# CHONSPQX/modulated-deform-conv

Measured on AMD Instinct MI355X. Metric: fwd+bwd GSamples/s, MDCN2d 3x3 C=256 56x56 B=32; %HBM roofline, higher is better.
Workload: dtype f32; 1 GPU; ModulatedDeformConv2d 3x3, C_in=C_out=256, 56x56, deformable_group=1, fp32, B=32 per GPU, forward+backward (BASELINE.json configs[1]); global_batch=32, parallelism=dp1 batch-sharded

## Files before the change

modulated_deform_conv_amd/csrc/mfma_bwd_data.hip:

```cpp
#include "mfma_kernels.hpp"
#include "mfma_tile.hpp"
#include <algorithm>
#include <map>
#include <mutex>
#include <stdio.h>
#include <stdlib.h>
#include <type_traits>

namespace mdconv {

namespace {

int grid_for(int64_t total) {
  int64_t b = (total + 255) / 256;
  return (int)(b > 8192 ? 8192 : (b < 1 ? 1 : b));
}

__device__ __forceinline__ void pack_wq_items(const Geom &g, int ochunks, int cblks, const float *__restrict__ w,
                                              float *__restrict__ wq, int64_t first, int64_t step) {
  const int64_t total = (int64_t)g.K * ochunks * cblks * 2 * 64;
  for (int64_t i = first; i < total; i += step) {
    int64_t r = i;
    const int lane = (int)(r & 63); r >>= 6;
    const int q = (int)(r & 1); r >>= 1;
// ... 12 lines not shown
    reinterpret_cast<float4 *>(wq)[i] = make_float4(v[0], v[1], v[2], v[3]);
  }
}

__global__ __launch_bounds__(256) void pack_wq_kernel(Geom g, int ochunks, int cblks,
                                                      const float *__restrict__ w,
                                                      float *__restrict__ wq) {
  pack_wq_items(g, ochunks, cblks, w, wq, (int64_t)blockIdx.x * 256 + threadIdx.x, (int64_t)gridDim.x * 256);
}

__global__ __launch_bounds__(256) void bwd_prep_kernel(Geom g, int ochunks, int cblks, const float *__restrict__ w,
                                                       float *__restrict__ wq, int *__restrict__ cnt, int64_t cnt_n,
                                                       const float *__restrict__ x, float *__restrict__ xt,
                                                       int nb_pack, int nb_zero, int qtiles, int ctiles) {
  __shared__ float t[32][33];
  int bid = blockIdx.x;
  if (bid < nb_pack) {
    pack_wq_items(g, ochunks, cblks, w, wq, (int64_t)bid * 256 + threadIdx.x, (int64_t)nb_pack * 256);
    return;
  }
  bid -= nb_pack;
  if (bid < nb_zero) {
    for (int64_t i = (int64_t)bid * 256 + threadIdx.x; i < cnt_n; i += (int64_t)nb_zero * 256) cnt[i] = 0;
    return;
  }
  bid -= nb_zero;
  const int qx = bid % qtiles, cy = (bid / qtiles) % ctiles, b = bid / (qtiles * ctiles);
  nchw_to_nhwc_tile(t, g.C, g.S_i, x, xt, b, cy * 32, qx * 32);
}




template <int ND, bool MOD, int WAVES_C, int QPQ, bool CL, typename GP = GeomRuntime>
__global__ __launch_bounds__(256, 2) void mfma_bwd_data_kernel(
    Geom g_arg, BwdDims bd, const float *__restrict__ input, const float *__restrict__ gout,
    const float *__restrict__ wq, const float *__restrict__ offset, const float *__restrict__ mask,
    float *__restrict__ gcol, float *__restrict__ grad_offset, float *__restrict__ grad_mask,
    float *__restrict__ ga, float *__restrict__ bias_part, int *__restrict__ cnt,
    int *__restrict__ table, const float *__restrict__ xt, int ntiles, int n_full, int n_tail, int tpw) {
  constexpr int NC = 1 << ND, NP = NC / 2;
  constexpr int MB = 2;
  constexpr int WAVES_P = 4 / WAVES_C;
  constexpr int BNP = 32 * WAVES_P;
  constexpr int RB = ND == 2 ? 8 : 4;
  constexpr int NBATCH = MB * 16 / RB;
  constexpr int HS = NBATCH / 2, CPS = NC / HS;
  constexpr int kOob = 0x7ffffff0;
  static_assert(!GP::kFixed || (ND == 2 && MOD && QPQ > 0), "the canonical geometry is 2-D, modulated, one conv group");
  const auto &g = GP::view(g_arg);
  extern __shared__ __attribute__((aligned(16))) float smem[];
  const int T_o = bd.ochunks;
  const int gpitch = T_o * 16 + 4;
  float *Gs = smem;
  float *red = smem + BNP * gpitch;
  const int kTapGroup = bd.tap_group;

  const int tid = threadIdx.x, lane = tid & 63, kh = lane >> 5;
  const int wave = __builtin_amdgcn_readfirstlane(tid >> 6);
  const int wc = wave / WAVES_P, wp = wave % WAVES_P;

  int u0, u1;
  if ((int)blockIdx.x < n_full) {
    u0 = xcd_remap(blockIdx.x, n_full) * g.K * tpw;
    u1 = u0 + g.K * tpw;
  } else {
    const int j = xcd_remap(blockIdx.x - n_full, n_tail);
    const int64_t tail_units = (int64_t)(ntiles - n_full * tpw) * g.K;
    u0 = n_full * tpw * g.K + (int)(tail_units * j / n_tail);
    u1 = n_full * tpw * g.K + (int)(tail_units * (j + 1) / n_tail);
  }
  if (u0 >= u1) return;

  const int passes = bd.cblks_q / (2 * WAVES_C);
  const int iters = (u1 - u0) * passes;
  const int nquads = T_o / 4;
  const bool per_block = g.DG > 1;
  const int nblk = per_block ? passes * WAVES_C : WAVES_C;
  const int bpd = per_block ? g.Cdg / 64 : nblk;
  const int frag_bytes = 64 * 16;
  const int chunk_bytes = bd.cblks_q * 2 * frag_bytes;
  const rsrc_t r_in = make_rsrc(CL ? xt : input, (size_t)g.B * g.C * g.S_i * 4);
  const rsrc_t r_wq = make_rsrc(wq, (size_t)g.K * T_o * chunk_bytes);
  const rsrc_t r_gc = make_rsrc(gcol, (size_t)g.B * g.C * g.K * g.S_o * 4);
  const int a_lane = lane * 16;
  const float *Bb = Gs + (wp * 32 + (lane & 31)) * gpitch + 4 * kh;
  constexpr int kStRow = 2 * NC + 4;
  float *Pk = red + bd.red_floats + wave * (32 * 64);
  int *St = reinterpret_cast<int *>(red + bd.red_floats + 4 * 32 * 64) + wave * (32 * kStRow);
  const int gl_p = lane >> 2, gl_j = lane & 3;
  auto pk_swz = [](int p) { return ((p & 3) << 2) | ((p >> 2) & 3); };
  if (CL) {
    for (int i = lane; i < 32 * 64; i += 64) Pk[i] = 0.f;
    for (int i = lane; i < 32 * kStRow; i += 64) St[i] = kOob;
  }

  auto krange = [&](int pass, int &q_lo, int &q_n) {
    if (g.G == 1) { q_lo = 0; q_n = nquads; return; }
    const int cb = (pass * WAVES_C + wc) * 64;
    const int c_lo = min(cb, g.C - 1), c_hi = min(cb + 63, g.C - 1);
    const int o_lo = (c_lo / g.Cg) * g.Og, o_hi = (c_hi / g.Cg + 1) * g.Og;
    q_lo = o_lo / 64;
    q_n = (o_hi + 63) / 64 - q_lo;
  };
  auto a_base = [&](int tap, int pass, int q_lo) {
    return (tap * T_o + q_lo * 4) * chunk_bytes + ((pass * WAVES_C + wc) * 2) * 2 * frag_bytes;
  };
  int a_cur = 0, n_cur = 0, a_nxt = 0, b_cur = 0;
  auto a_off = [&](int t) { return t < n_cur ? a_cur + t * chunk_bytes : a_nxt + (t - n_cur) * chunk_bytes; };
  auto load_a = [&](float4 (&ra)[MB][2], int soff) {
#pragma unroll
    for (int i = 0; i < MB; ++i)
#pragma unroll
      for (int q = 0; q < 2; ++q)
        ra[i][q] = buf_load4(r_wq, a_lane + (i * 2 + q) * frag_bytes, soff);
  };
  float4 ra0[MB][2], ra1[MB][2], ra2[MB][2], ra3[MB][2];
  {
    int q_lo, q_n;
    krange(0, q_lo, q_n);
    a_cur = a_base(u0 % g.K, 0, q_lo);
    n_cur = 4;
    load_a(ra0, a_off(0));
    load_a(ra1, a_off(1));
    load_a(ra2, a_off(2));
  }

  struct Pix { int n0, b, pix; bool live; int oc[ND]; };
  auto pix_of_tile = [&](int tile, Pix &px) {
    px.n0 = tile * BNP;
    const int n_raw = px.n0 + wp * 32 + (lane & 31);
    px.live = n_raw < g.N;
    const int n_l = px.live ? n_raw : g.N - 1;
    px.b = n_l / g.S_o;
    px.pix = n_l - px.b * g.S_o;
    out_coords<ND>(g, px.pix, px.oc);
  };
  Pix pc, pp;
  pix_of_tile(u0 / g.K, pc);
  pp = pc;

  auto load_gout_tile = [&](int tile) {
    const int j = tid % BNP, osub = tid / BNP;
    constexpr int OSTEP = 256 / BNP;
    const int n_t = min(tile * BNP + j, g.N - 1);
    const int b_t = n_t / g.S_o, pix_t = n_t - b_t * g.S_o;
    const bool t_live = tile * BNP + j < g.N;
    const float *src = gout + ((int64_t)b_t * g.O) * g.S_o + pix_t;
    float *dst = Gs + j * gpitch;
    const int Opad = T_o * 16;
#pragma unroll 8
    for (int o = osub; o < Opad; o += OSTEP) {
      const float v = src[(int64_t)min(o, g.O - 1) * g.S_o];
      dst[o] = (t_live && o < g.O) ? v : 0.f;
    }
  };

  constexpr int PGS = BNP / 4;
  constexpr int OPR = 256 / PGS;
  constexpr int kPre = 8;
  const bool gout_vec = (g.S_o & 3) == 0 && (reinterpret_cast<uintptr_t>(gout) & 15) == 0;
  auto load_gout_tile_vec = [&](int tile) {
    const int Opad = T_o * 16;
    const int rounds = (Opad + OPR - 1) / OPR;
    const int j4 = (tid % PGS) * 4;
    const bool live4 = tile * BNP + j4 < g.N;
    const int n4 = min(tile * BNP + j4, g.N - 4);
    const int b4 = n4 / g.S_o, pix4 = n4 - b4 * g.S_o;
    const float *src = gout + ((int64_t)b4 * g.O) * g.S_o + pix4;
    const int o0 = tid / PGS;
    float *dst = Gs + j4 * gpitch + o0;
    for (int r0 = 0; r0 < rounds; r0 += kPre) {
      float4 v[kPre];
#pragma unroll
      for (int i = 0; i < kPre; ++i)
        v[i] = *reinterpret_cast<const float4 *>(src + (int64_t)min((r0 + i) * OPR + o0, g.O - 1) * g.S_o);
#pragma unroll
      for (int i = 0; i < kPre; ++i) {
        const int o = (r0 + i) * OPR + o0;
        if (o < Opad) {
          const bool on = live4 && o < g.O;
          float *d = dst + (r0 + i) * OPR;
          d[0] = on ? v[i].x : 0.f;
          d[gpitch] = on ? v[i].y : 0.f;
          d[2 * gpitch] = on ? v[i].z : 0.f;
          d[3 * gpitch] = on ? v[i].w : 0.f;
        }
      }
    }
  };

  auto emit_ga = [&](int tile) {
    constexpr int NCH = BNP / 16;
    const int Opad = T_o * 16;
    const int total = NCH * bd.mblks * 2 * 64;
    for (int i = tid; i < total; i += 256) {
      int r = i;
      const int ln = r & 63; r >>= 6;
      const int q = r & 1; r >>= 1;
      const int mblk = r % bd.mblks, nch = r / bd.mblks;
      const int nchunk = tile * NCH + nch;
      if (nchunk * 16 >= bd.Np) continue;
      const int o = mblk * 32 + (ln & 31);
      const float *src = Gs + (nch * 16 + 8 * q + 4 * (ln >> 5)) * gpitch + o;
      float4 v = make_float4(0.f, 0.f, 0.f, 0.f);
      if (o < Opad) v = make_float4(src[0], src[gpitch], src[2 * gpitch], src[3 * gpitch]);
      reinterpret_cast<float4 *>(ga)[((int64_t)nchunk * bd.mblks + mblk) * 128 + q * 64 + ln] = v;
    }
    if (bias_part != nullptr)
      for (int o = tid; o < g.O; o += 256) {
        float sacc = 0.f;
#pragma unroll 8
        for (int px = 0; px < BNP; ++px) sacc += Gs[px * gpitch + o];
        bias_part[(int64_t)tile * g.O + o] = sacc;
      }
  };

  int voff[NP], gc_voff = kOob;
  int voffc[NC];
  struct Fac { float ol[ND - 1], oh[ND - 1], osl[ND - 1], osh[ND - 1], xw, yw, xs, ys; } fac;
  float mg = 0.f;
  float S[NC];
  float delta_n[ND], m_n = 1.f;
  typedef unsigned long long lanemask_t;
  lanemask_t bad[NC];
#pragma unroll
  for (int ci = 0; ci < NC; ++ci) bad[ci] = 0ull;
  f32x16 acc[MB], accp[MB];
#pragma unroll
  for (int pi = 0; pi < NP; ++pi) voff[pi] = kOob;
#pragma unroll
  for (int ci = 0; ci < NC; ++ci) voffc[ci] = kOob;
#pragma unroll
  for (int ci = 0; ci < NC; ++ci) S[ci] = 0.f;
#pragma unroll
  for (int a = 0; a < ND; ++a) delta_n[a] = 0.f;
#pragma unroll
  for (int a = 0; a < ND - 1; ++a) fac.ol[a] = fac.oh[a] = fac.osl[a] = fac.osh[a] = 0.f;
  fac.xw = fac.yw = fac.xs = fac.ys = 0.f;
#pragma unroll
  for (int i = 0; i < MB; ++i)
#pragma unroll
    for (int r = 0; r < 16; ++r) accp[i][r] = 0.f;

  auto new_tap_state = [&](int tapp, int dgp, bool count) {
    int tcd[ND];
    tap_coords<ND>(g, tapp, tcd);
    TapCoef<ND, float> tc;
    make_tap<ND, float>(g, pp.oc, tcd, delta_n, true, tc);
    mg = (!g.range_gate || tc.inside) ? m_n : 0.f;
    int pidx[NP];
    float px[NP], py[NP];
    make_pairs<ND, float>(g, tc, 1.f, pidx, px, py);
    bool prx[NP], pry[NP];
    make_pairs_read<ND, float>(g, tc, prx, pry);
    if (ND == 3 && count && kh == 0 && pp.live) {
      SampleAnchor<ND> sa;
      sample_anchor<ND>(g, tc, 1.f, sa);
      if (sa.on) atomicAdd(cnt + ((int64_t)pp.b * g.DG + dgp) * bd.S_e + sa.qa, 1);
    }
    if (ND == 2 && count && kh == 0 && pp.live) {
      int aidx[NP];
      float ax[NP], ay[NP];
      make_pairs_f<ND, float>(g, tc, tc.wl, tc.wha, 1.f, aidx, ax, ay);
      int *cseg = cnt + ((int64_t)pp.b * g.DG + dgp) * g.S_i;
#pragma unroll
      for (int pi = 0; pi < NP; ++pi)
        if (ax[pi] != 0.f || ay[pi] != 0.f) atomicAdd(cseg + aidx[pi], 1);
    }
    if (count && kh == 0) {
      const int n = pp.n0 + wp * 32 + lane;
      if (n < bd.Np) {
        int *e = table + ((int64_t)(dgp * g.K + tapp) * bd.Np + n) * (2 * NC);
        int ev[2 * NC];
#pragma unroll
        for (int pi = 0; pi < NP; ++pi) {
          if (bd.cl) {
            ev[2 * pi] = pp.live && prx[pi] ? (pp.b * g.S_i + pidx[pi]) * g.C * 4 : kOob;
// ... 21 lines not shown
      }
      voffc[2 * pi] = prx[pi] ? (pp.b * g.S_i + pidx[pi]) * g.C * 4 + 16 * kh : kOob;
      voffc[2 * pi + 1] = pry[pi] ? (pp.b * g.S_i + pidx[pi] + 1) * g.C * 4 + 16 * kh : kOob;
    }
    {
      constexpr int L = ND - 1;
      const int lc = tc.last_lc, hc = tc.last_lc + tc.delta[L];
      const int cl = min(lc, g.in_sz[L] - 2);
      fac.xw = (lc == cl ? tc.wl[L] : 0.f) + (hc == cl ? tc.wh[L] : 0.f);
      fac.yw = (lc == cl + 1 ? tc.wl[L] : 0.f) + (hc == cl + 1 ? tc.wh[L] : 0.f);
      fac.xs = (lc == cl ? tc.sl[L] : 0.f) + (hc == cl ? tc.sh[L] : 0.f);
      fac.ys = (lc == cl + 1 ? tc.sl[L] : 0.f) + (hc == cl + 1 ? tc.sh[L] : 0.f);
#pragma unroll
      for (int a = 0; a < L; ++a) { fac.ol[a] = tc.wl[a]; fac.oh[a] = tc.wh[a]; fac.osl[a] = tc.sl[a]; fac.osh[a] = tc.sh[a]; }
    }
    gc_voff = pp.live ? ((((pp.b * g.K + tapp) * g.S_o + pp.pix) * g.C) + 4 * kh) * 4 : kOob;
    if (CL && kh == 0) {
      int *st = St + lane * kStRow;
#pragma unroll
      for (int c4 = 0; c4 < NC; c4 += 4)
        *reinterpret_cast<int4 *>(st + c4) = make_int4(voffc[c4], voffc[c4 + 1], voffc[c4 + 2], voffc[c4 + 3]);
      st[NC] = gc_voff;
    }
#pragma unroll
    for (int ci = 0; ci < NC; ++ci) S[ci] = 0.f;
  };

  struct Batch { float f[RB * NC]; };
  auto gather = [&](int q, int cbase_p, Batch &v) {
    const int mb = (q * RB) / 16, r0 = (q * RB) % 16;
    if (CL) {
      const int pxl = (q / HS) * 16 + gl_p;
      const int *st = St + pxl * kStRow + (q % HS) * CPS;
      const bool full = cbase_p + 64 <= g.C;
      if (full) {
#pragma unroll
        for (int c = 0; c < CPS; ++c) {
          const int o = st[c] + 16 * gl_j;
#pragma unroll
          for (int k = 0; k < 4; ++k) {
            const float4 x = buf_load4(r_in, o + 64 * k, cbase_p * 4);
            float *d = v.f + (c * 4 + k) * 4;
            d[0] = x.x; d[1] = x.y; d[2] = x.z; d[3] = x.w;
          }
        }
      } else {
#pragma unroll
        for (int c = 0; c < CPS; ++c) {
          const int o = st[c] + 16 * gl_j;
#pragma unroll
          for (int k = 0; k < 4; ++k) {
            const float4 x = buf_load4(r_in, cbase_p + 16 * k + 4 * gl_j < g.C ? o + 64 * k : kOob, cbase_p * 4);
            float *d = v.f + (c * 4 + k) * 4;
            d[0] = x.x; d[1] = x.y; d[2] = x.z; d[3] = x.w;
          }
        }
      }
    } else {
#pragma unroll
      for (int rr = 0; rr < RB; ++rr) {
        const int r = r0 + rr;
        const int cu = cbase_p + mb * 32 + (r & 3) + 8 * (r >> 2);
        const int cs = min(cu, g.C - 5) * g.S_i * 4;
#pragma unroll
        for (int pi = 0; pi < NP; ++pi) {
          const float2 x = buf_load2(r_in, voff[pi], cs);
          v.f[(rr * NP + pi) * 2] = x.x;
          v.f[(rr * NP + pi) * 2 + 1] = x.y;
        }
      }
    }
  };
  auto consume = [&](int q, int cbase_p, const Batch &v) {
    if (CL) {
      const int pxl = (q / HS) * 16 + gl_p, cp = q % HS;
      int *st = St + pxl * kStRow;
      const int swz = pk_swz(pxl);
      const bool full = cbase_p + 64 <= g.C;
      float4 gc[4];
#pragma unroll
      for (int k = 0; k < 4; ++k)
        gc[k] = *reinterpret_cast<const float4 *>(Pk + pxl * 64 + 4 * ((4 * k + gl_j) ^ swz));
      if (cp == 0) {
        const int gv = st[NC] + 16 * gl_j;
#pragma unroll
        for (int k = 0; k < 4; ++k)
          buf_store4(r_gc, (full || cbase_p + 16 * k + 4 * gl_j < g.C) ? gv + 64 * k : kOob, cbase_p * 4,
                     gc[k].x, gc[k].y, gc[k].z, gc[k].w);
      }
      float s[CPS];
#pragma unroll
      for (int c = 0; c < CPS; ++c) {
        float a = 0.f;
#pragma unroll
        for (int k = 0; k < 4; ++k) {
          const float *x = v.f + (c * 4 + k) * 4;
          a = fmaf(gc[k].w, x[3], fmaf(gc[k].z, x[2], fmaf(gc[k].y, x[1], fmaf(gc[k].x, x[0], a))));
        }
        s[c] = a;
      }
      static_assert(CPS == 2, "two corners per step");
      asm("s_nop 1\n\t"
          "v_add_f32_dpp %0, %0, %0 quad_perm:[1,0,3,2] row_mask:0xf bank_mask:0xf\n\t"
          "v_add_f32_dpp %1, %1, %1 quad_perm:[1,0,3,2] row_mask:0xf bank_mask:0xf\n\t"
          "s_nop 1\n\t"
          "v_add_f32_dpp %0, %0, %0 quad_perm:[2,3,0,1] row_mask:0xf bank_mask:0xf\n\t"
          "v_add_f32_dpp %1, %1, %1 quad_perm:[2,3,0,1] row_mask:0xf bank_mask:0xf\n\t"
          "s_nop 1"
          : "+v"(s[0]), "+v"(s[1]));
      if (gl_j == 0) *reinterpret_cast<float2 *>(st + NC + 4 + cp * CPS) = make_float2(s[0], s[1]);
      return;
    }
    const int mb = (q * RB) / 16, r0 = (q * RB) % 16;
#pragma unroll
    for (int gq = 0; gq < RB / 4; ++gq) {
      const int cu4 = cbase_p + mb * 32 + 8 * ((r0 >> 2) + gq);
      const int vo = cu4 < g.C ? gc_voff : kOob;
      buf_store4(r_gc, vo, cu4 * 4, accp[mb][r0 + 4 * gq], accp[mb][r0 + 4 * gq + 1],
                 accp[mb][r0 + 4 * gq + 2], accp[mb][r0 + 4 * gq + 3]);
    }
    lanemask_t any_bad = 0ull;
#pragma unroll
    for (int ci = 0; ci < NC; ++ci) any_bad |= bad[ci];
    if (any_bad != 0ull) {
#pragma unroll
      for (int rr = 0; rr < RB; ++rr) {
        const float gc = accp[mb][r0 + rr];
#pragma unroll
        for (int ci = 0; ci < NC; ++ci) {
          float x;
          asm("v_cndmask_b32_e64 %0, %1, 0, %2" : "=v"(x) : "v"(v.f[(rr * NP + (ci >> 1)) * 2 + (ci & 1)]), "s"(bad[ci]));
          S[ci] = fmaf(gc, x, S[ci]);
        }
      }
    } else {
#pragma unroll
      for (int rr = 0; rr < RB; ++rr) {
        const float gc = accp[mb][r0 + rr];
#pragma unroll
        for (int ci = 0; ci < NC; ++ci) {
          const float x = v.f[(rr * NP + (ci >> 1)) * 2 + (ci & 1)];
          S[ci] = fmaf(gc, x, S[ci]);
        }
      }
    }
#pragma unroll
    for (int ci = 0; ci < NC; ++ci) asm volatile("" : "+v"(S[ci]));
  };

  auto collect = [&]() {
    if (CL) {
      const float *sr = reinterpret_cast<const float *>(St + (lane & 31) * kStRow + NC + 4);
#pragma unroll
      for (int c4 = 0; c4 < NC; c4 += 4) {
        const float4 t = *reinterpret_cast<const float4 *>(sr + c4);
        S[c4] += t.x; S[c4 + 1] += t.y; S[c4 + 2] += t.z; S[c4 + 3] += t.w;
      }
    }
  };
  auto park = [&]() {
    if (CL) {
      const int pix = lane & 31, swz = pk_swz(pix);
      float *dst = Pk + pix * 64;
#pragma unroll
      for (int i = 0; i < MB; ++i)
#pragma unroll
        for (int rq = 0; rq < 4; ++rq)
          *reinterpret_cast<float4 *>(dst + 4 * ((i * 8 + 2 * rq + kh) ^ swz)) =
              make_float4(acc[i][4 * rq], acc[i][4 * rq + 1], acc[i][4 * rq + 2], acc[i][4 * rq + 3]);
    } else {
#pragma unroll
      for (int i = 0; i < MB; ++i) accp[i] = acc[i];
    }
  };

  int grp_lo = (u0 % g.K) % kTapGroup;
  auto finish_tap = [&](int tapp, int blk, bool flush_ok, bool last) {
    float goff[ND], gm = 0.f;
    {
      constexpr int L = ND - 1;
      float Tw[NP], Ts[NP];
#pragma unroll
      for (int pi = 0; pi < NP; ++pi) {
        Tw[pi] = fmaf(fac.xw, S[2 * pi], fac.yw * S[2 * pi + 1]);
        Ts[pi] = fmaf(fac.xs, S[2 * pi], fac.ys * S[2 * pi + 1]);
      }
#pragma unroll
      for (int a = 0; a < ND; ++a) goff[a] = 0.f;
#pragma unroll
      for (int pi = 0; pi < NP; ++pi) {
        float ow = 1.f;
#pragma unroll
        for (int a = 0; a < L; ++a) ow *= ((pi >> (L - 1 - a)) & 1) ? fac.oh[a] : fac.ol[a];
        gm = fmaf(ow, Tw[pi], gm);
        goff[L] = fmaf(ow, Ts[pi], goff[L]);
#pragma unroll
        for (int a = 0; a < L; ++a) {
          float od = 1.f;
#pragma unroll
          for (int a2 = 0; a2 < L; ++a2) {
            const bool hi = (pi >> (L - 1 - a2)) & 1;
            od *= (a2 == a) ? (hi ? fac.osh[a2] : fac.osl[a2]) : (hi ? fac.oh[a2] : fac.ol[a2]);
          }
          goff[a] = fmaf(od, Tw[pi], goff[a]);
        }
      }
#pragma unroll
      for (int a = 0; a < ND; ++a) goff[a] *= mg;
    }
    if (!CL) {
#pragma unroll
      for (int a = 0; a < ND; ++a) goff[a] += __shfl_xor(goff[a], 32, 64);
      gm += __shfl_xor(gm, 32, 64);
    }
    if (bd.red_floats == 0) {
      if (kh == 0 && pp.live) {
        const int64_t ob = ((int64_t)pp.b * (ND * g.K) + ND * tapp) * g.S_o + pp.pix;
#pragma unroll
        for (int a = 0; a < ND; ++a) {
          float *dst = grad_offset + ob + (int64_t)a * g.S_o;
          *dst = g.acc_data ? *dst + goff[a] : goff[a];
        }
        if (MOD) {
          float *dst = grad_mask + ((int64_t)pp.b * g.K + tapp) * g.S_o + pp.pix;
          *dst = g.acc_data ? *dst + gm : gm;
        }
      }
      return;
    }
    const int slot = tapp % kTapGroup;
    if (kh == 0) {
      float *rp = red + ((slot * nblk + blk) * (ND + 1)) * BNP + wp * 32 + lane;
#pragma unroll
      for (int a = 0; a < ND; ++a) rp[a * BNP] = goff[a];
      rp[ND * BNP] = gm;
    }
    if (flush_ok && (slot == kTapGroup - 1 || tapp == g.K - 1 || last)) {
      __syncthreads();
      const int tap0 = tapp - slot;
      const int per_slot = g.DG * (ND + 1) * BNP;
      const int items = (slot + 1 - grp_lo) * per_slot;
      for (int x = tid; x < items; x += 256) {
        const int jj = x % BNP, a = (x / BNP) % (ND + 1), dgi = (x / (BNP * (ND + 1))) % g.DG;
        const int sl = grp_lo + x / per_slot;
        const int n = pp.n0 + jj;
        if (n < g.N && (MOD || a < ND)) {
          float sum = 0.f;
          for (int y = 0; y < bpd; ++y)
            sum += red[((sl * nblk + dgi * bpd + y) * (ND + 1) + a) * BNP + jj];
          const int b = n / g.S_o, pix = n - b * g.S_o, tp = tap0 + sl;
          const int64_t seg = (int64_t)b * g.DG + dgi;
          float *dst = a < ND ? grad_offset + (seg * (ND * g.K) + ND * tp + a) * g.S_o + pix
                              : grad_mask + (seg * g.K + tp) * g.S_o + pix;
          *dst = g.acc_data ? *dst + sum : sum;
        }
      }
      __syncthreads();
      grp_lo = 0;
    }
  };

  auto mma = [&](const float4 (&ra)[MB][2], const float *bp, bool fresh) {
    const float4 b0 = *reinterpret_cast<const float4 *>(bp);
    const float4 b1 = *reinterpret_cast<const float4 *>(bp + 8);
    const f32x16 zero = {0.f, 0.f, 0.f, 0.f, 0.f, 0.f, 0.f, 0.f, 0.f, 0.f, 0.f, 0.f, 0.f, 0.f, 0.f, 0.f};
#pragma unroll
    for (int q = 0; q < 2; ++q)
#pragma unroll
      for (int s = 0; s < 4; ++s) {
        const float4 bq = q == 0 ? b0 : b1;
        const float b = s == 0 ? bq.x : (s == 1 ? bq.y : (s == 2 ? bq.z : bq.w));
#pragma unroll
        for (int i = 0; i < MB; ++i) {
          const float a = s == 0 ? ra[i][q].x : (s == 1 ? ra[i][q].y : (s == 2 ? ra[i][q].z : ra[i][q].w));
          acc[i] = __builtin_amdgcn_mfma_f32_32x32x2f32(a, b, (fresh && q == 0 && s == 0) ? zero : acc[i], 0, 0, 0);
        }
      }
  };
  auto quad_head = [&](int t) { load_a(ra3, a_off(t + 3)); };
  auto quad_tail = [&](int t, bool fresh) {
    const float *bq = Bb + b_cur;
    __builtin_amdgcn_sched_barrier(0);
    mma(ra0, bq + t * 16, fresh);
    load_a(ra0, a_off(t + 4));
    __builtin_amdgcn_sched_barrier(0);
    mma(ra1, bq + (t + 1) * 16, false);
    load_a(ra1, a_off(t + 5));
    __builtin_amdgcn_sched_barrier(0);
    mma(ra2, bq + (t + 2) * 16, false);
    load_a(ra2, a_off(t + 6));
    __builtin_amdgcn_sched_barrier(0);
    mma(ra3, bq + (t + 3) * 16, false);
  };
  auto quad = [&](int t, bool fresh) { quad_head(t); quad_tail(t, fresh); };

  int tile_c = -1;
  int tapp = 0, passp = 0;
  int tile = u0 / g.K, tap = u0 - tile * g.K, pass = 0;
  for (int it = 0; it < iters; ++it) {
    if (it > 0 && (passp == 0 || per_block)) {
      const int blk = passp * WAVES_C + wc;
      if (per_block) new_tap_state(tapp, min(blk * 64, g.C - 1) / g.Cdg, blk % bpd == 0 && blk * 64 < g.C);
      else new_tap_state(tapp, 0, wc == 0);
    }
    if (tile != tile_c) {
      if (tile_c >= 0) __syncthreads();
      if (gout_vec) load_gout_tile_vec(tile);
      else load_gout_tile(tile);
      pix_of_tile(tile, pc);
      tile_c = tile;
      __syncthreads();
      if (tap == 0 && pass == 0) emit_ga(tile);
    }
    if (pass == 0 || per_block) {
      const int dg = per_block ? min((pass * WAVES_C + wc) * 64, g.C - 1) / g.Cdg : 0;
      const int64_t seg = (int64_t)pc.b * g.DG + dg;
      const int64_t ob = (seg * (ND * g.K) + ND * tap) * g.S_o + pc.pix;
#pragma unroll
      for (int a = 0; a < ND; ++a) delta_n[a] = offset[ob + (int64_t)a * g.S_o];
      if (MOD) m_n = mask[(seg * g.K + tap) * g.S_o + pc.pix];
    }
    int nq;
    {
      int q_lo, tn = tap, pn = pass + 1;
      krange(pass, q_lo, nq);
      a_cur = a_base(tap, pass, q_lo);
      n_cur = nq * 4;
      b_cur = q_lo * 64;
      if (pn == passes) { pn = 0; tn = tap + 1 == g.K ? 0 : tap + 1; }
      int q_lo2, nq2;
      krange(pn, q_lo2, nq2);
      a_nxt = a_base(tn, pn, q_lo2);
    }
    const int cbase_p = (passp * WAVES_C + wc) * 64;
    if (QPQ == 0) {
#pragma unroll
      for (int i = 0; i < MB; ++i)
#pragma unroll
        for (int r = 0; r < 16; ++r) acc[i][r] = 0.f;
    }

#pragma unroll
    for (int q = 0; q < NBATCH; ++q) {
      Batch v;
      if (QPQ > 0) quad_head(q * QPQ * 4);
      gather(q, cbase_p, v);
      asm volatile("" ::: "memory");
      __builtin_amdgcn_sched_barrier(0);
      if (QPQ > 0) {
        quad_tail(q * QPQ * 4, q == 0);
#pragma unroll
        for (int jq = 1; jq < QPQ; ++jq) quad((q * QPQ + jq) * 4, false);
      } else {
        for (int qd = nq * q / NBATCH; qd < nq * (q + 1) / NBATCH; ++qd) quad(qd * 4, false);
      }
      __builtin_amdgcn_sched_barrier(0);
      consume(q, cbase_p, v);
      asm volatile("" ::: "memory");
      __builtin_amdgcn_sched_barrier(0);
    }
    collect();
    if (it > 0 && (passp == passes - 1 || per_block))
      finish_tap(tapp, per_block ? passp * WAVES_C + wc : wc, passp == passes - 1, false);
    park();
    pp = pc;
    tapp = tap;
    passp = pass;
    if (++pass == passes) {
      pass = 0;
      if (++tap == g.K) { tap = 0; ++tile; }
    }
  }
  {
    if (passp == 0 || per_block) {
      const int blk = passp * WAVES_C + wc;
      if (per_block) new_tap_state(tapp, min(blk * 64, g.C - 1) / g.Cdg, blk % bpd == 0 && blk * 64 < g.C);
      else new_tap_state(tapp, 0, wc == 0);
    }
    const int cbase_p = (passp * WAVES_C + wc) * 64;
    static_assert(NBATCH % 2 == 0, "pairs of drain batches");
#pragma unroll
    for (int q = 0; q < NBATCH; q += 2) {
      Batch v0, v1;
      gather(q, cbase_p, v0);
      gather(q + 1, cbase_p, v1);
      asm volatile("" ::: "memory");
      __builtin_amdgcn_sched_barrier(0);
      consume(q, cbase_p, v0);
      consume(q + 1, cbase_p, v1);
      asm volatile("" ::: "memory");
      __builtin_amdgcn_sched_barrier(0);
    }
    collect();
    finish_tap(tapp, per_block ? passp * WAVES_C + wc : wc, true, true);
  }
}


template <int ND, bool MOD>
__global__ __launch_bounds__(256) void csr_fill_kernel(Geom g, const float *__restrict__ offset,
                                                       const float *__restrict__ mask,
                                                       int *__restrict__ cursor,
                                                       const int *__restrict__ rowptr,
                                                       int4 *__restrict__ entries) {
  constexpr int NP = 1 << (ND - 1);
  const int64_t total = (int64_t)g.B * g.DG * g.K * g.S_o;
  for (int64_t i = (int64_t)blockIdx.x * 256 + threadIdx.x; i < total; i += (int64_t)gridDim.x * 256) {
    const int pix = (int)(i % g.S_o);
    const int tap = (int)((i / g.S_o) % g.K);
    const int seg = (int)(i / g.S_o / g.K);
// ... 101 lines not shown
                                     hipFuncAttributeMaxDynamicSharedMemorySize, (int)kBwdDataLdsCap); \
    });                                                                                         \
    if (attr_err != hipSuccess) { set_error("hipFuncSetAttribute: %s", hipGetErrorString(attr_err)); return MDCONV_ELAUNCH; } \
     \
     \
    int occ_q = 0;                                                                              \
    {                                                                                           \
      static std::mutex occ_mu;                                                                 \
      static std::map<size_t, int> occ_by_lds;                                                  \
      std::lock_guard<std::mutex> lock(occ_mu);                                                 \
      auto it = occ_by_lds.find(lds);                                                           \
      if (it == occ_by_lds.end()) {                                                             \
        int nq = 0;                                                                             \
        (void)hipOccupancyMaxActiveBlocksPerMultiprocessor(                                     \
            &nq, (const void *)mfma_bwd_data_kernel<ND, MOD, WC, QPQ, CL, GP>, 256, lds);           \
        (void)hipGetLastError();                                                                \
        it = occ_by_lds.emplace(lds, nq > 0 ? nq : (lds * 2 <= 160 * 1024 ? 2 : 1)).first;      \
      }                                                                                         \
      occ_q = it->second;                                                                       \
    }                                                                                           \
    const int slots = num_cus() * occ_q;                                                        \
    const int tpw = 2;                        \
    const int n_full = ntiles / (slots * tpw) * slots;                                          \
    static const bool debug_plan = getenv("MDCONV_DEBUG_PLAN") != nullptr;                      \
    if (debug_plan)                                                                             \
      fprintf(stderr, "[mdconv] GEMM-1 plan: %d tiles, %zu B LDS, %d resident per CU\n", ntiles, lds, occ_q); \
    if (debug_plan)                                                                             \
      fprintf(stderr, "[mdconv] GEMM-1 instance <%d,%d,%d,%d,%d>, geometry: %s\n", ND, (int)MOD, WC, QPQ, (int)CL, \
              GP::kFixed ? "canonical 3x3 (compile-time)" : "run-time");                       \
    note_geometry_variant(GP::kFixed ? 1 : 0);                                                  \
    const int n_tail = (int)std::min<int64_t>((int64_t)(ntiles - n_full * tpw) * g.K, slots);   \
    hipLaunchKernelGGL((mfma_bwd_data_kernel<ND, MOD, WC, QPQ, CL, GP>), dim3(n_full + n_tail), \
                       dim3(256), lds, stream,                                                  \
                       g, bd, (const float *)t.input, (const float *)t.grad_output, wq,         \
                       (const float *)t.offset, (const float *)t.mask, gcol,                    \
                       (float *)t.grad_offset, (float *)t.grad_mask, ga, bias_part, cnt, table, xt,        \
                       ntiles, n_full, n_tail, tpw);                                            \
  } while (0)
                                                \
#define LAUNCH_BD(ND, MOD, WC, QPQ)                                                             \
  do {                                                                                          \
    if (xt != nullptr && bd.cl_drain) LAUNCH_BD_(ND, MOD, WC, QPQ, true, GeomRuntime);          \
    else LAUNCH_BD_(ND, MOD, WC, QPQ, false, GeomRuntime);                                      \
  } while (0)
 \
#define LAUNCH_BD_Q(ND, MOD, WC, QPQ)                                                           \
  do {                                                                                          \
     \
    using GPc = std::conditional<(ND == 2 && MOD && (QPQ) > 0), GeomCanon3x3, GeomRuntime>::type; \
    if (GPc::kFixed && geom_canon3x3_selected(g)) {                                             \
      if (xt != nullptr && bd.cl_drain) LAUNCH_BD_(ND, MOD, WC, QPQ, true, GPc);                \
      else LAUNCH_BD_(ND, MOD, WC, QPQ, false, GPc);                                            \
    } else {                                                                                    \
      LAUNCH_BD(ND, MOD, WC, QPQ);                                                              \
    }                                                                                           \
  } while (0)
#define LAUNCH_BD2(ND, MOD)                                                                     \
  do {                                                                                          \
    const int nbatch = ND == 2 ? 4 : 8, nquads = bd.ochunks / 4;                                \
                   \
    const int qpq = (ND == 2 && g.G == 1 && nquads % nbatch == 0 && nquads / nbatch <= 2) ? nquads / nbatch : 0; \
    if (bd.waves_c == 4) {                                                                      \
      if (ND == 2 && qpq == 1) LAUNCH_BD_Q(ND, MOD, 4, (ND == 2 ? 1 : 0));                      \
      else if (ND == 2 && qpq == 2) LAUNCH_BD_Q(ND, MOD, 4, (ND == 2 ? 2 : 0));                 \
      else LAUNCH_BD(ND, MOD, 4, 0);                                                            \
    } else if (bd.waves_c == 2) LAUNCH_BD(ND, MOD, 2, 0);                                       \
    else LAUNCH_BD(ND, MOD, 1, 0);                                                              \
  } while (0)
  if (g.nd == 2) { if (g.modulated) LAUNCH_BD2(2, true); else LAUNCH_BD2(2, false); }
  else { if (g.modulated) LAUNCH_BD2(3, true); else LAUNCH_BD2(3, false); }
// ... 32 lines not shown
```

modulated_deform_conv_amd/csrc/mfma_tile.hpp:

```cpp
#pragma once
#include "mdconv_common.hpp"

namespace mdconv {

typedef float f32x16 __attribute__((ext_vector_type(16)));

constexpr int kBK = 16;

struct PackDims {
  int Cgp;
  int Ogp;
  int BM;
};

inline PackDims pack_dims(const Geom &g) {
  PackDims pd;
  pd.BM = g.Og > 128 ? 256 : (g.Og > 64 ? 128 : 64);
  pd.Cgp = (g.Cg + 2 * kBK - 1) / (2 * kBK) * (2 * kBK);
  pd.Ogp = (g.Og + pd.BM - 1) / pd.BM * pd.BM;
  return pd;
}

__device__ __forceinline__ int xcd_remap(int bid, int n) {
  const int q = n >> 3, r = n & 7;
// ... 22 lines not shown
}

template <int AUX = 0>
__device__ __forceinline__ void buf_store4(rsrc_t r, int voff, int soff, float a, float b, float c,
                                           float d) {
  typedef unsigned int u32x4 __attribute__((__vector_size__(4 * sizeof(unsigned int))));
  const u32x4 v = {__builtin_bit_cast(unsigned, a), __builtin_bit_cast(unsigned, b),
                   __builtin_bit_cast(unsigned, c), __builtin_bit_cast(unsigned, d)};
  __builtin_amdgcn_raw_buffer_store_b128(v, r, voff, soff, AUX);
}

struct BwdDims {
  int Np;
  int cl;
  int wtile;
  int OgpB, mblks, mtiles;
  int Cp, cblks;
  int splits, pairs_per_split;
  int ochunks;
  int waves_c, cblks_q;
  int bias_tiles;
  int red_floats;
  int tap_group;
  int cl_drain;
  int sample_keyed;
  int S_e;
  size_t off_wq, off_ga, off_table, off_part, off_gcol, off_cnt, off_rowptr, off_entries, off_bias,
      off_xt, off_sums, off_bstage, off_sort, off_end;
  int two_pass;
};
BwdDims bwd_dims(const Geom &g, Skip skip = Skip());

#ifdef __HIPCC__
__device__ __forceinline__ void nchw_to_nhwc_tile(float (*t)[33], int C, int S, const float *__restrict__ x,
                                                  float *__restrict__ xt, int b, int c0, int q0) {
  const int tx = threadIdx.x & 31, ty = threadIdx.x >> 5;
  const float *src = x + ((size_t)b * C + c0) * S;
  float *dst = xt + ((size_t)b * S + q0) * C + c0;
#pragma unroll
  for (int r = ty; r < 32; r += 8) t[r][tx] = (q0 + tx < S) ? src[(size_t)r * S + q0 + tx] : 0.f;
  __syncthreads();
#pragma unroll
  for (int r = ty; r < 32; r += 8)
    if (q0 + r < S) dst[(size_t)r * C + tx] = t[tx][r];
}
#endif

int pack_weights_f32(const Geom &g, const PackDims &pd, const float *weight, float *wp, float *wq,
                     hipStream_t stream);
size_t fwd_tail_bytes(const Geom &g);
constexpr int kTailMaxPerCu = 5;
void fwd_tail_plan(const Geom &g, int tiles, int slots, int *full_tiles, int *ways, int *n_hi);
int fwd_tail_reduce_launch(int BM, int BN, const Geom &g, const float *part, const float *bias, float *output, int ntm,
                           int tail_tiles, int full_tiles, int ways, int n_hi, hipStream_t stream);
int mfma_forward_f32(const Geom &g, const PackDims &pd, const Tensors &t, const float *wp, float *part,
                     hipStream_t stream);
bool geom_canon3x3_selected(const Geom &g);
bool fwd_channels_last(const Geom &g);
size_t fwd_cl_bytes(const Geom &g);
int mfma_forward_cl_f32(const Geom &g, const PackDims &pd, const Tensors &t, const float *wp, float *part,
                        float *xt, hipStream_t stream);
int mfma_bwd_weight_f32(const Geom &g, const BwdDims &bd, const Tensors &t, const float *ga,
                        const int *table, float *part, const float *bias_part, const float *xt,
                        hipStream_t stream);
int mfma_bwd_weight_cl_launch(const Geom &g, const BwdDims &bd, const float *xt, const float *ga,
                              const int *table, float *part, hipStream_t stream);
// ... 29 lines not shown
```

Measured before the change: 73.47 GSamples/s.

## Reread kernel args from kernarg segment to cut SGPR pressure in bwd-data kernel

Packs the bwd-data kernel parameters into one struct and, instead of keeping them live in scalar registers, re-reads them from the kernarg segment pointer at each use site behind an opaque asm barrier. The A-fragment offset is also made a running scalar counter when the output-chunk count is a compile-time constant, and the tile/gout load is moved before the tap-state update. The aim is to lower scalar register pressure and spills in the main loop, at the cost of extra scalar memory loads of the arguments.

```diff
diff --git a/modulated_deform_conv_amd/csrc/mfma_bwd_data.hip b/modulated_deform_conv_amd/csrc/mfma_bwd_data.hip
--- a/modulated_deform_conv_amd/csrc/mfma_bwd_data.hip
+++ b/modulated_deform_conv_amd/csrc/mfma_bwd_data.hip
@@ -68,13 +68,19 @@
 
 
 
+
+struct Gemm1Args {
+  Geom g;
+  BwdDims bd;
+  const float *input, *gout, *wq, *offset, *mask;
+  float *gcol, *grad_offset, *grad_mask, *ga, *bias_part;
+  int *cnt, *table;
+  const float *xt;
+  int ntiles, n_full, n_tail, tpw;
+};
+
 template <int ND, bool MOD, int WAVES_C, int QPQ, bool CL, typename GP = GeomRuntime>
-__global__ __launch_bounds__(256, 2) void mfma_bwd_data_kernel(
-    Geom g_arg, BwdDims bd, const float *__restrict__ input, const float *__restrict__ gout,
-    const float *__restrict__ wq, const float *__restrict__ offset, const float *__restrict__ mask,
-    float *__restrict__ gcol, float *__restrict__ grad_offset, float *__restrict__ grad_mask,
-    float *__restrict__ ga, float *__restrict__ bias_part, int *__restrict__ cnt,
-    int *__restrict__ table, const float *__restrict__ xt, int ntiles, int n_full, int n_tail, int tpw) {
+__global__ __launch_bounds__(256, 2) void mfma_bwd_data_kernel(Gemm1Args) {
   constexpr int NC = 1 << ND, NP = NC / 2;
   constexpr int MB = 2;
   constexpr int WAVES_P = 4 / WAVES_C;
@@ -84,46 +90,50 @@
   constexpr int HS = NBATCH / 2, CPS = NC / HS;
   constexpr int kOob = 0x7ffffff0;
   static_assert(!GP::kFixed || (ND == 2 && MOD && QPQ > 0), "the canonical geometry is 2-D, modulated, one conv group");
-  const auto &g = GP::view(g_arg);
   extern __shared__ __attribute__((aligned(16))) float smem[];
-  const int T_o = bd.ochunks;
+  const Gemm1Args *kp0 = kernarg_reread<Gemm1Args>();
+  const auto &g0 = GP::view(kp0->g);
+  const int K = g0.K, C = g0.C;
+  const int T_o = QPQ > 0 ? QPQ * NBATCH * 4 : kp0->bd.ochunks;
   const int gpitch = T_o * 16 + 4;
   float *Gs = smem;
   float *red = smem + BNP * gpitch;
-  const int kTapGroup = bd.tap_group;
 
   const int tid = threadIdx.x, lane = tid & 63, kh = lane >> 5;
   const int wave = __builtin_amdgcn_readfirstlane(tid >> 6);
   const int wc = wave / WAVES_P, wp = wave % WAVES_P;
 
   int u0, u1;
-  if ((int)blockIdx.x < n_full) {
-    u0 = xcd_remap(blockIdx.x, n_full) * g.K * tpw;
-    u1 = u0 + g.K * tpw;
-  } else {
-    const int j = xcd_remap(blockIdx.x - n_full, n_tail);
-    const int64_t tail_units = (int64_t)(ntiles - n_full * tpw) * g.K;
-    u0 = n_full * tpw * g.K + (int)(tail_units * j / n_tail);
-    u1 = n_full * tpw * g.K + (int)(tail_units * (j + 1) / n_tail);
+  {
+    const int n_full = kp0->n_full, n_tail = kp0->n_tail, tpw = kp0->tpw;
+    if ((int)blockIdx.x < n_full) {
+      u0 = xcd_remap(blockIdx.x, n_full) * K * tpw;
+      u1 = u0 + K * tpw;
+    } else {
+      const int j = xcd_remap(blockIdx.x - n_full, n_tail);
+      const int64_t tail_units = (int64_t)(kp0->ntiles - n_full * tpw) * K;
+      u0 = n_full * tpw * K + (int)(tail_units * j / n_tail);
+      u1 = n_full * tpw * K + (int)(tail_units * (j + 1) / n_tail);
+    }
   }
   if (u0 >= u1) return;
 
-  const int passes = bd.cblks_q / (2 * WAVES_C);
+  const int passes = kp0->bd.cblks_q / (2 * WAVES_C);
   const int iters = (u1 - u0) * passes;
   const int nquads = T_o / 4;
-  const bool per_block = g.DG > 1;
-  const int nblk = per_block ? passes * WAVES_C : WAVES_C;
-  const int bpd = per_block ? g.Cdg / 64 : nblk;
+  const bool per_block = g0.DG > 1;
   const int frag_bytes = 64 * 16;
-  const int chunk_bytes = bd.cblks_q * 2 * frag_bytes;
-  const rsrc_t r_in = make_rsrc(CL ? xt : input, (size_t)g.B * g.C * g.S_i * 4);
-  const rsrc_t r_wq = make_rsrc(wq, (size_t)g.K * T_o * chunk_bytes);
-  const rsrc_t r_gc = make_rsrc(gcol, (size_t)g.B * g.C * g.K * g.S_o * 4);
+  const int chunk_bytes = kp0->bd.cblks_q * 2 * frag_bytes;
+  const int S_i4 = CL ? 0 : g0.S_i * 4;
+  const int red_floats = kp0->bd.red_floats;
+  const rsrc_t r_in = make_rsrc(CL ? kp0->xt : kp0->input, (size_t)g0.B * g0.C * g0.S_i * 4);
+  const rsrc_t r_wq = make_rsrc(kp0->wq, (size_t)g0.K * T_o * chunk_bytes);
+  const rsrc_t r_gc = make_rsrc(kp0->gcol, (size_t)g0.B * g0.C * g0.K * g0.S_o * 4);
   const int a_lane = lane * 16;
   const float *Bb = Gs + (wp * 32 + (lane & 31)) * gpitch + 4 * kh;
   constexpr int kStRow = 2 * NC + 4;
-  float *Pk = red + bd.red_floats + wave * (32 * 64);
-  int *St = reinterpret_cast<int *>(red + bd.red_floats + 4 * 32 * 64) + wave * (32 * kStRow);
+  float *Pk = red + red_floats + wave * (32 * 64);
+  int *St = reinterpret_cast<int *>(red + red_floats + 4 * 32 * 64) + wave * (32 * kStRow);
   const int gl_p = lane >> 2, gl_j = lane & 3;
   auto pk_swz = [](int p) { return ((p & 3) << 2) | ((p >> 2) & 3); };
   if (CL) {
@@ -131,8 +141,8 @@
     for (int i = lane; i < 32 * kStRow; i += 64) St[i] = kOob;
   }
 
-  auto krange = [&](int pass, int &q_lo, int &q_n) {
-    if (g.G == 1) { q_lo = 0; q_n = nquads; return; }
+  auto krange = [&](const Geom &g, int pass, int &q_lo, int &q_n) {
+    if (QPQ > 0 || g.G == 1) { q_lo = 0; q_n = nquads; return; }
     const int cb = (pass * WAVES_C + wc) * 64;
     const int c_lo = min(cb, g.C - 1), c_hi = min(cb + 63, g.C - 1);
     const int o_lo = (c_lo / g.Cg) * g.Og, o_hi = (c_hi / g.Cg + 1) * g.Og;
@@ -143,7 +153,17 @@
     return (tap * T_o + q_lo * 4) * chunk_bytes + ((pass * WAVES_C + wc) * 2) * 2 * frag_bytes;
   };
   int a_cur = 0, n_cur = 0, a_nxt = 0, b_cur = 0;
-  auto a_off = [&](int t) { return t < n_cur ? a_cur + t * chunk_bytes : a_nxt + (t - n_cur) * chunk_bytes; };
+  int a_run = 0;
+  auto a_off = [&](int t) {
+    if (QPQ > 0) {
+      if (t == T_o) a_run = a_nxt;
+      const int so = a_run;
+      a_run += chunk_bytes;
+      asm("" : "+s"(a_run));
+      return so;
+    }
+    return t < n_cur ? a_cur + t * chunk_bytes : a_nxt + (t - n_cur) * chunk_bytes;
+  };
   auto load_a = [&](float4 (&ra)[MB][2], int soff) {
 #pragma unroll
     for (int i = 0; i < MB; ++i)
@@ -154,8 +174,9 @@
   float4 ra0[MB][2], ra1[MB][2], ra2[MB][2], ra3[MB][2];
   {
     int q_lo, q_n;
-    krange(0, q_lo, q_n);
-    a_cur = a_base(u0 % g.K, 0, q_lo);
+    krange(g0, 0, q_lo, q_n);
+    a_cur = a_base(u0 % K, 0, q_lo);
+    a_run = a_cur;
     n_cur = 4;
     load_a(ra0, a_off(0));
     load_a(ra1, a_off(1));
@@ -163,7 +184,7 @@
   }
 
   struct Pix { int n0, b, pix; bool live; int oc[ND]; };
-  auto pix_of_tile = [&](int tile, Pix &px) {
+  auto pix_of_tile = [&](const Geom &g, int tile, Pix &px) {
     px.n0 = tile * BNP;
     const int n_raw = px.n0 + wp * 32 + (lane & 31);
     px.live = n_raw < g.N;
@@ -173,10 +194,10 @@
     out_coords<ND>(g, px.pix, px.oc);
   };
   Pix pc, pp;
-  pix_of_tile(u0 / g.K, pc);
+  pix_of_tile(g0, u0 / K, pc);
   pp = pc;
 
-  auto load_gout_tile = [&](int tile) {
+  auto load_gout_tile = [&](const Geom &g, const float *gout, int tile) {
     const int j = tid % BNP, osub = tid / BNP;
     constexpr int OSTEP = 256 / BNP;
     const int n_t = min(tile * BNP + j, g.N - 1);
@@ -195,8 +216,7 @@
   constexpr int PGS = BNP / 4;
   constexpr int OPR = 256 / PGS;
   constexpr int kPre = 8;
-  const bool gout_vec = (g.S_o & 3) == 0 && (reinterpret_cast<uintptr_t>(gout) & 15) == 0;
-  auto load_gout_tile_vec = [&](int tile) {
+  auto load_gout_tile_vec = [&](const Geom &g, const float *gout, int tile) {
     const int Opad = T_o * 16;
     const int rounds = (Opad + OPR - 1) / OPR;
     const int j4 = (tid % PGS) * 4;
@@ -226,8 +246,10 @@
     }
   };
 
-  auto emit_ga = [&](int tile) {
+  auto emit_ga = [&](const Gemm1Args *kp, const Geom &g, int tile) {
     constexpr int NCH = BNP / 16;
+    const BwdDims &bd = kp->bd;
+    float *ga = kp->ga, *bias_part = kp->bias_part;
     const int Opad = T_o * 16;
     const int total = NCH * bd.mblks * 2 * 64;
     for (int i = tid; i < total; i += 256) {
@@ -279,7 +301,9 @@
 #pragma unroll
     for (int r = 0; r < 16; ++r) accp[i][r] = 0.f;
 
-  auto new_tap_state = [&](int tapp, int dgp, bool count) {
+  auto new_tap_state = [&](const Gemm1Args *kp, const Geom &g, int tapp, int dgp, bool count) {
+    const BwdDims &bd = kp->bd;
+    int *cnt = kp->cnt, *table = kp->table;
     int tcd[ND];
     tap_coords<ND>(g, tapp, tcd);
     TapCoef<ND, float> tc;
@@ -367,7 +391,7 @@
     if (CL) {
       const int pxl = (q / HS) * 16 + gl_p;
       const int *st = St + pxl * kStRow + (q % HS) * CPS;
-      const bool full = cbase_p + 64 <= g.C;
+      const bool full = cbase_p + 64 <= C;
       if (full) {
 #pragma unroll
         for (int c = 0; c < CPS; ++c) {
@@ -385,7 +409,7 @@
           const int o = st[c] + 16 * gl_j;
 #pragma unroll
           for (int k = 0; k < 4; ++k) {
-            const float4 x = buf_load4(r_in, cbase_p + 16 * k + 4 * gl_j < g.C ? o + 64 * k : kOob, cbase_p * 4);
+            const float4 x = buf_load4(r_in, cbase_p + 16 * k + 4 * gl_j < C ? o + 64 * k : kOob, cbase_p * 4);
             float *d = v.f + (c * 4 + k) * 4;
             d[0] = x.x; d[1] = x.y; d[2] = x.z; d[3] = x.w;
           }
@@ -396,7 +420,7 @@
       for (int rr = 0; rr < RB; ++rr) {
         const int r = r0 + rr;
         const int cu = cbase_p + mb * 32 + (r & 3) + 8 * (r >> 2);
-        const int cs = min(cu, g.C - 5) * g.S_i * 4;
+        const int cs = min(cu, C - 5) * S_i4;
 #pragma unroll
         for (int pi = 0; pi < NP; ++pi) {
           const float2 x = buf_load2(r_in, voff[pi], cs);
@@ -411,7 +435,7 @@
       const int pxl = (q / HS) * 16 + gl_p, cp = q % HS;
       int *st = St + pxl * kStRow;
       const int swz = pk_swz(pxl);
-      const bool full = cbase_p + 64 <= g.C;
+      const bool full = cbase_p + 64 <= C;
       float4 gc[4];
 #pragma unroll
       for (int k = 0; k < 4; ++k)
@@ -420,7 +444,7 @@
         const int gv = st[NC] + 16 * gl_j;
 #pragma unroll
         for (int k = 0; k < 4; ++k)
-          buf_store4(r_gc, (full || cbase_p + 16 * k + 4 * gl_j < g.C) ? gv + 64 * k : kOob, cbase_p * 4,
+          buf_store4(r_gc, (full || cbase_p + 16 * k + 4 * gl_j < C) ? gv + 64 * k : kOob, cbase_p * 4,
                      gc[k].x, gc[k].y, gc[k].z, gc[k].w);
       }
       float s[CPS];
@@ -450,7 +474,7 @@
 #pragma unroll
     for (int gq = 0; gq < RB / 4; ++gq) {
       const int cu4 = cbase_p + mb * 32 + 8 * ((r0 >> 2) + gq);
-      const int vo = cu4 < g.C ? gc_voff : kOob;
+      const int vo = cu4 < C ? gc_voff : kOob;
       buf_store4(r_gc, vo, cu4 * 4, accp[mb][r0 + 4 * gq], accp[mb][r0 + 4 * gq + 1],
                  accp[mb][r0 + 4 * gq + 2], accp[mb][r0 + 4 * gq + 3]);
     }
@@ -509,8 +533,14 @@
     }
   };
 
-  int grp_lo = (u0 % g.K) % kTapGroup;
+  int grp_lo = (u0 % K) % kp0->bd.tap_group;
   auto finish_tap = [&](int tapp, int blk, bool flush_ok, bool last) {
+    const Gemm1Args *kp = kernarg_reread<Gemm1Args>();
+    const auto &g = GP::view(kp->g);
+    const int kTapGroup = kp->bd.tap_group;
+    const int nblk = per_block ? passes * WAVES_C : WAVES_C;
+    const int bpd = per_block ? g.Cdg / 64 : nblk;
+    float *grad_offset = kp->grad_offset, *grad_mask = kp->grad_mask;
     float goff[ND], gm = 0.f;
     {
       constexpr int L = ND - 1;
@@ -548,7 +578,7 @@
       for (int a = 0; a < ND; ++a) goff[a] += __shfl_xor(goff[a], 32, 64);
       gm += __shfl_xor(gm, 32, 64);
     }
-    if (bd.red_floats == 0) {
+    if (red_floats == 0) {
       if (kh == 0 && pp.live) {
         const int64_t ob = ((int64_t)pp.b * (ND * g.K) + ND * tapp) * g.S_o + pp.pix;
 #pragma unroll
@@ -570,7 +600,7 @@
       for (int a = 0; a < ND; ++a) rp[a * BNP] = goff[a];
       rp[ND * BNP] = gm;
     }
-    if (flush_ok && (slot == kTapGroup - 1 || tapp == g.K - 1 || last)) {
+    if (flush_ok && (slot == kTapGroup - 1 || tapp == K - 1 || last)) {
       __syncthreads();
       const int tap0 = tapp - slot;
       const int per_slot = g.DG * (ND + 1) * BNP;
@@ -631,26 +661,34 @@
 
   int tile_c = -1;
   int tapp = 0, passp = 0;
-  int tile = u0 / g.K, tap = u0 - tile * g.K, pass = 0;
+  int tile = u0 / K, tap = u0 - tile * K, pass = 0;
   for (int it = 0; it < iters; ++it) {
+    if (tile != tile_c) {
+      const Gemm1Args *kt = kernarg_reread<Gemm1Args>();
+      const auto &gt = GP::view(kt->g);
+      if (tile_c >= 0) __syncthreads();
+      const float *gout = kt->gout;
+      const bool gout_vec = (gt.S_o & 3) == 0 && (reinterpret_cast<uintptr_t>(gout) & 15) == 0;
+      if (gout_vec) load_gout_tile_vec(gt, gout, tile);
+      else load_gout_tile(gt, gout, tile);
+      pix_of_tile(gt, tile, pc);
+      tile_c = tile;
+      __syncthreads();
+      if (tap == 0 && pass == 0) emit_ga(kt, gt, tile);
+    }
+    const Gemm1Args *kp = kernarg_reread<Gemm1Args>();
+    const auto &g = GP::view(kp->g);
     if (it > 0 && (passp == 0 || per_block)) {
       const int blk = passp * WAVES_C + wc;
-      if (per_block) new_tap_state(tapp, min(blk * 64, g.C - 1) / g.Cdg, blk % bpd == 0 && blk * 64 < g.C);
-      else new_tap_state(tapp, 0, wc == 0);
-    }
-    if (tile != tile_c) {
-      if (tile_c >= 0) __syncthreads();
-      if (gout_vec) load_gout_tile_vec(tile);
-      else load_gout_tile(tile);
-      pix_of_tile(tile, pc);
-      tile_c = tile;
-      __syncthreads();
-      if (tap == 0 && pass == 0) emit_ga(tile);
+      const int bpd = per_block ? g.Cdg / 64 : WAVES_C;
+      if (per_block) new_tap_state(kp, g, tapp, min(blk * 64, C - 1) / g.Cdg, blk % bpd == 0 && blk * 64 < C);
+      else new_tap_state(kp, g, tapp, 0, wc == 0);
     }
     if (pass == 0 || per_block) {
-      const int dg = per_block ? min((pass * WAVES_C + wc) * 64, g.C - 1) / g.Cdg : 0;
+      const int dg = per_block ? min((pass * WAVES_C + wc) * 64, C - 1) / g.Cdg : 0;
       const int64_t seg = (int64_t)pc.b * g.DG + dg;
       const int64_t ob = (seg * (ND * g.K) + ND * tap) * g.S_o + pc.pix;
+      const float *offset = kp->offset, *mask = kp->mask;
 #pragma unroll
       for (int a = 0; a < ND; ++a) delta_n[a] = offset[ob + (int64_t)a * g.S_o];
       if (MOD) m_n = mask[(seg * g.K + tap) * g.S_o + pc.pix];
@@ -658,13 +696,14 @@
     int nq;
     {
       int q_lo, tn = tap, pn = pass + 1;
-      krange(pass, q_lo, nq);
+      krange(g, pass, q_lo, nq);
       a_cur = a_base(tap, pass, q_lo);
+      a_run = a_cur + 3 * chunk_bytes;
       n_cur = nq * 4;
       b_cur = q_lo * 64;
-      if (pn == passes) { pn = 0; tn = tap + 1 == g.K ? 0 : tap + 1; }
+      if (pn == passes) { pn = 0; tn = tap + 1 == K ? 0 : tap + 1; }
       int q_lo2, nq2;
-      krange(pn, q_lo2, nq2);
+      krange(g, pn, q_lo2, nq2);
       a_nxt = a_base(tn, pn, q_lo2);
     }
     const int cbase_p = (passp * WAVES_C + wc) * 64;
@@ -703,14 +742,17 @@
     passp = pass;
     if (++pass == passes) {
       pass = 0;
-      if (++tap == g.K) { tap = 0; ++tile; }
+      if (++tap == K) { tap = 0; ++tile; }
     }
   }
   {
     if (passp == 0 || per_block) {
+      const Gemm1Args *kp = kernarg_reread<Gemm1Args>();
+      const auto &g = GP::view(kp->g);
       const int blk = passp * WAVES_C + wc;
-      if (per_block) new_tap_state(tapp, min(blk * 64, g.C - 1) / g.Cdg, blk % bpd == 0 && blk * 64 < g.C);
-      else new_tap_state(tapp, 0, wc == 0);
+      const int bpd = per_block ? g.Cdg / 64 : WAVES_C;
+      if (per_block) new_tap_state(kp, g, tapp, min(blk * 64, C - 1) / g.Cdg, blk % bpd == 0 && blk * 64 < C);
+      else new_tap_state(kp, g, tapp, 0, wc == 0);
     }
     const int cbase_p = (passp * WAVES_C + wc) * 64;
     static_assert(NBATCH % 2 == 0, "pairs of drain batches");
@@ -878,10 +920,10 @@
     const int n_tail = (int)std::min<int64_t>((int64_t)(ntiles - n_full * tpw) * g.K, slots);   \
     hipLaunchKernelGGL((mfma_bwd_data_kernel<ND, MOD, WC, QPQ, CL, GP>), dim3(n_full + n_tail), \
                        dim3(256), lds, stream,                                                  \
-                       g, bd, (const float *)t.input, (const float *)t.grad_output, wq,         \
-                       (const float *)t.offset, (const float *)t.mask, gcol,                    \
-                       (float *)t.grad_offset, (float *)t.grad_mask, ga, bias_part, cnt, table, xt,        \
-                       ntiles, n_full, n_tail, tpw);                                            \
+                       Gemm1Args{g, bd, (const float *)t.input, (const float *)t.grad_output, wq, \
+                                 (const float *)t.offset, (const float *)t.mask, gcol,          \
+                                 (float *)t.grad_offset, (float *)t.grad_mask, ga, bias_part, cnt, table, xt, \
+                                 ntiles, n_full, n_tail, tpw});                                 \
   } while (0)
                                                 \
 #define LAUNCH_BD(ND, MOD, WC, QPQ)                                                             \
diff --git a/modulated_deform_conv_amd/csrc/mfma_tile.hpp b/modulated_deform_conv_amd/csrc/mfma_tile.hpp
--- a/modulated_deform_conv_amd/csrc/mfma_tile.hpp
+++ b/modulated_deform_conv_amd/csrc/mfma_tile.hpp
@@ -78,6 +78,12 @@
 BwdDims bwd_dims(const Geom &g, Skip skip = Skip());
 
 #ifdef __HIPCC__
+template <typename T> __device__ __forceinline__ const T *kernarg_reread() {
+  auto p = __builtin_amdgcn_kernarg_segment_ptr();
+  asm volatile("" : "+s"(p));
+  return (const T *)p;
+}
+
 __device__ __forceinline__ void nchw_to_nhwc_tile(float (*t)[33], int C, int S, const float *__restrict__ x,
                                                   float *__restrict__ xt, int b, int c0, int q0) {
   const int tx = threadIdx.x & 31, ty = threadIdx.x >> 5;
```

Result: no change. 73.52 GSamples/s (median of 4 runs) (+0.1%).
